# deep-art-project/Music

Measured on AMD Instinct MI355X. Metric: audio samples/sec trained (whole node), 30-layer WaveNet @16kHz, higher is better.
Workload: dtype f32 (forward + recompute: f16 2-term split operands, 2^-22 per element; backward products: bf16 2-term split, 2^-17 per element, f32 range; 3 MFMA per product, f32 accumulate)

## Files before the change

### include/wavenet_hip.h

```cpp
#ifndef WAVENET_HIP_H
#define WAVENET_HIP_H
#include <stdint.h>
#ifdef __cplusplus
extern "C" {
#endif

typedef void* wn_stream_t;
enum { WN_F16X3 = 0, WN_F16X1 = 1, WN_BF16X3 = 2, WN_BF16X1 = 3 };
#define WN_ABI_VERSION 5
#define WN_CE_NUM_PARTIALS 1024

int wn_version(void);
const char* wn_last_error(void);

int wn_pack_weights(const float* flat, const int32_t* idx, uint16_t* out, int n, int mode,
                    wn_stream_t stream);

int wn_chan_gemm(const float* in0, const float* in1, int64_t in_bstride, int in_pitch, int in_lo, int in_hi,
                 int shift0, int shift1, int ks0, int ks1, const uint16_t* wpack, int mt, int m_valid,
                 float* out, int64_t out_bstride, int out_pitch, int out_shift, const float* bias,
                 const float* resid, int64_t resid_bstride, int resid_pitch, int resid_lo,
                 const float* mask, int64_t mask_bstride, int mask_pitch,
                 int t_lo, int t_hi, int relu_in, int batch, int mode, wn_stream_t stream);

int wn_resblock_fwd(const float* x_in, float* x_out, float* z_out, int64_t x_bstride, int64_t z_bstride,
                    int pitch, const uint16_t* wfg, const uint16_t* wd, const float* bias_f,
                    const float* bias_g, const float* bias_d, int n_f, int n_d, int ch, int d,
                    int t_lo, int t_hi, int z_lo, int write_x, const float* cond, int64_t cond_bstride,
                    int cond_pitch, int cond_mode, int cond_le, int cond_q, const uint16_t* cond_pack,
                    int64_t cond_pack_bstride, const uint8_t* cond_idx, int64_t z_half_stride, int batch, int mode,
                    wn_stream_t stream);

int wn_resblock_bwd(const float* x_in, const float* dy, const float* dz, float* dfg, float* z,
                    int64_t x_bstride, int64_t dz_bstride, int64_t dfg_bstride, int64_t z_bstride,
                    int pitch, const uint16_t* wfg, const uint16_t* wdT, const float* bias_f,
                    const float* bias_g, int n_f, int ch, int d, int t_lo, int t_hi, int z_lo,
                    const float* cond, int64_t cond_bstride, int cond_pitch, int cond_mode, int cond_le, int cond_q,
                    int batch, int mode_fwd, int mode_bwd, wn_stream_t stream);

int wn_skip_epilogue_fwd(const float* z, int64_t z_bstride, int pitch, int ks_skip, const uint16_t* w_skip, const float* bias_skip,
                         float* u, float* h, int64_t s_bstride, const uint16_t* w_p1c, const float* bias_p1,
                         const uint16_t* w_p2c, const float* bias_p2, float* o, int64_t o_bstride, int o_pitch,
// ... 26 lines not shown
int wn_resblock_bwd_ms_slabs(int t_lo, int t_hi, int batch);

#define WN_COND_IDX_PAD 64
int wn_resblock_bwd_pq(const float* x_in, const float* p_in, const float* q_in, int dn, int p_lo, const float* dz,
                       float* p_out, float* q_out, int64_t x_bstride, int64_t dz_bstride, int pitch, const uint16_t* wfg,
                       const uint16_t* wdT, const uint16_t* wpq, int ch, int d, int t_lo, int t_hi, int z_lo,
                       float* slab_fg, float* slab_d, const float* cond, int64_t cond_bstride, int cond_pitch, int cond_le,
                       const uint8_t* cond_idx, float* cslab, int64_t dz_half_stride, int chain, int batch, int mode_fwd,
                       int mode_bwd, wn_stream_t stream);
int wn_resblock_bwd_pq_chain_ok(int t_lo, int t_hi, int batch, int d);
int wn_resblock_bwd_pq_slabs(int t_lo, int t_hi, int batch, int d, int chain);
int wn_resblock_bwd_pq_chain_items(int t_lo, int t_hi, int batch, int d, int wg, int* out, int cap);
int wn_resblock_bwd_pq_cond_floats(int t_lo, int t_hi, int batch);
int wn_resblock_bwd_pq_cond_reduce(const float* cslab, const int64_t* slab_off, const int* t_lo, int n_launches, int t_hi, int batch,
                                   int cond_le, float* out, int64_t out_lstride, int64_t out_bstride, int out_pitch,
                                   wn_stream_t stream);
int wn_gate_fwd(const float* fg, int64_t fg_bstride, int dp, int rows, float* z, int64_t z_bstride, int pitch, int t_lo, int t_hi,
                int batch, wn_stream_t stream);
int wn_gate_bwd(const float* fg, int64_t fg_bstride, int dp, int rows, const float* dz, int64_t dz_bstride, float* dfg,
                int64_t dfg_bstride, int pitch, int t_lo, int t_hi, int batch, wn_stream_t stream);
int wn_chunk_softmax_fwd(const float* x, float* y, int64_t nrows, int q, wn_stream_t stream);
int wn_chunk_softmax_bwd(const float* y, const float* dy, float* dx, int64_t nrows, int q, wn_stream_t stream);
int wn_chunk_softmax_ce(const float* x, const int64_t* target, float* probs, float* dx, float* loss_part, int64_t nrows, int q,
                        float inv_n, wn_stream_t stream);
int wn_split16(const float* x, uint16_t* hi, uint16_t* lo, int64_t n, int is_bf16, wn_stream_t stream);
int wn_shift_add(const float* p, const float* q, float* out, int64_t bstride, int pitch, int rows, int dn, int p_lo,
                 int t_lo, int t_hi, int batch, wn_stream_t stream);

int wn_wgrad(const float* a, int64_t a_bstride, int a_pitch, int a_shift, int a_cols,
             const float* b0, const float* b1, int64_t b_bstride, int b_pitch, int b_shift0,
             int b_shift1, int b_cols, int nt_per_tap, int mt, int relu_b, float* c, int ldc,
             int64_t c_slab_stride, int t_lo, int t_hi, int chunk, int batch, int mode, wn_stream_t stream);
int wn_wgrad_slabs(int t_lo, int t_hi, int chunk, int batch);
int wn_causal_wgrad_codes(const int32_t* codes, int scrambled, const float* dx, const float* dx_q, int dn, int p_lo,
                          int64_t dx_bstride, int pitch, int ch, int q, int t, int batch, float* slab, wn_stream_t stream);
int wn_causal_wgrad_codes_slabs(int t, int batch);
int wn_causal_fwd_codes(const int32_t* codes, int scrambled, const float* wt, const float* bias, int n_rows, float* x0,
                        int64_t x_bstride, int pitch, int ch, int q, int t, int batch, wn_stream_t stream);
int wn_reduce_slabs(const int64_t* desc, int n_ops, int64_t total_vec, const float* slab, float* out,
                    wn_stream_t stream);

int wn_bias_grad(const float* a, int64_t a_bstride, int a_pitch, int a_shift, int rows, int t_lo,
                 int t_hi, int batch, float* out, wn_stream_t stream);

int wn_chunk_softmax256_fwd(const float* x, float* y, int64_t nrows, wn_stream_t stream);
int wn_chunk_softmax256_bwd(const float* y, const float* dy, float* dx, int64_t nrows, wn_stream_t stream);
int wn_chunk_softmax256_ce(const float* x, const int64_t* target, float* probs, float* dx,
                           float* loss_part, int64_t nrows, float inv_n, wn_stream_t stream);

int wn_adam_flat(float* p, const float* g, float* m, float* v, int64_t n, float lr, float beta1,
                 float beta2, float eps, float bias_corr1, float bias_corr2, float gscale,
                 wn_stream_t stream);
int wn_sgd_flat(float* p, const float* g, float* momentum_buf, int64_t n, float lr, float momentum, float gscale,
                int first_step, wn_stream_t stream);
int wn_rmsprop_flat(float* p, const float* g, float* square_avg, float* momentum_buf, int64_t n, float lr, float alpha,
                    float eps, float momentum, float gscale, wn_stream_t stream);
int wn_coll_available(void);
int wn_comm_unique_id(char* id128);
int wn_comm_create(int nranks, int rank, const char* id128, void** comm);
int wn_comm_destroy(void* comm);
int wn_allreduce_flat(void* comm, float* buf, int64_t n, wn_stream_t stream);
int wn_gather_grads(const float* packed, const int32_t* idx, float* flat_grad, int n, wn_stream_t stream);
int wn_gather_grads2(const float* packed, const int32_t* idx, const int32_t* idx2, float* flat_grad, int n, wn_stream_t stream);

int wn_cond_expand(const float* tab, int64_t tab_bstride, int tab_pitch, int rows, int t_lo, int t_hi, int mode, int le, int q,
                   float* out, int64_t out_bstride, int out_pitch, int batch, wn_stream_t stream);
// ... 44 lines not shown
```

### music_amd/_lib.py

```python
import ctypes
import os

_HERE = os.path.dirname(os.path.abspath(__file__))
LIB_PATH = os.environ.get("WAVENET_HIP_LIB") or os.path.join(_HERE, "libwavenet_hip.so")

F16X3, F16X1, BF16X3, BF16X1 = 0, 1, 2, 3
MODE_NAMES = {"f16x3": F16X3, "f16x1": F16X1, "bf16x3": BF16X3, "bf16x1": BF16X1}
CE_NUM_PARTIALS = 1024
ABI_VERSION = 5

_p = ctypes.c_void_p
_i = ctypes.c_int
_l = ctypes.c_int64
_f = ctypes.c_float

SIGNATURES = {
    "wn_version": [],
    "wn_pack_weights": [_p, _p, _p, _i, _i, _p],
    "wn_chan_gemm": [_p, _p, _l, _i, _i, _i, _i, _i, _i, _i, _p, _i, _i,
                     _p, _l, _i, _i, _p,
                     _p, _l, _i, _i,
                     _p, _l, _i,
                     _i, _i, _i, _i, _i, _p],
    "wn_skip_epilogue_fwd": [_p, _l, _i, _i, _p, _p, _p, _p, _l, _p, _p, _p, _p, _p, _l, _i, _i, _i, _i, _i, _i, _i, _p],
    "wn_skip_epilogue_bwd": [_p, _l, _i, _p, _p, _l, _i, _p, _p, _p, _l, _p, _p, _p, _i, _i, _i, _i, _i, _i, _i, _p],
    "wn_resblock_fwd": [_p, _p, _p, _l, _l, _i, _p, _p, _p, _p, _p, _i, _i, _i, _i,
                        _i, _i, _i, _i, _p, _l, _i, _i, _i, _i, _p, _l, _p, _l, _i, _i, _p],
    "wn_enc_resblock_fwd": [_p, _p, _p, _l, _l, _i, _p, _p, _p, _p, _i, _i, _i, _i, _i, _i, _i, _i, _p],
    "wn_enc_resblock_bwd": [_p, _p, _p, _p, _l, _l, _l, _i, _p, _i, _i, _i, _i, _i, _p, _p, _i, _i, _p],
    "wn_enc_resblock_bwd_slabs": [_i, _i, _i],
    "wn_enc_resblock_bwd_pq": [_p, _p, _p, _i, _i, _p, _p, _p, _l, _l, _i, _p, _p, _i, _i, _i, _i, _p, _p, _i, _i, _i, _p],
    "wn_avgpool": [_p, _l, _i, _i, _i, _i, _i, _p, _l, _i, _i, _p],
    "wn_resblock_bwd": [_p, _p, _p, _p, _p, _l, _l, _l, _l, _i, _p, _p, _p, _p, _i, _i, _i, _i, _i, _i,
                        _p, _l, _i, _i, _i, _i, _i, _i, _i, _p],
    "wn_cond_expand": [_p, _l, _i, _i, _i, _i, _i, _i, _i, _p, _l, _i, _i, _p],
    "wn_cond_grad": [_p, _l, _i, _i, _i, _i, _i, _i, _i, _p, _l, _i, _i, _p],
    "wn_avgpool_bwd": [_p, _l, _i, _i, _i, _i, _i, _p, _l, _i, _i, _i, _p],
    "wn_wgrad": [_p, _l, _i, _i, _i, _p, _p, _l, _i, _i, _i, _i, _i, _i, _i, _p, _i,
                 _l, _i, _i, _i, _i, _i, _p],
    "wn_wgrad_slabs": [_i, _i, _i, _i],
    "wn_resblock_bwd_ms": [_p, _p, _p, _p, _l, _l, _l, _i, _p, _p, _p, _p, _i, _i, _i, _i, _i, _i, _p, _p,
                           _p, _l, _i, _i, _i, _i, _i, _i, _i, _p],
    "wn_resblock_bwd_ms_slabs": [_i, _i, _i],
    "wn_resblock_bwd_pq": [_p, _p, _p, _i, _i, _p, _p, _p, _l, _l, _i, _p, _p, _p, _i, _i, _i, _i, _i, _p, _p,
                           _p, _l, _i, _i, _p, _p, _l, _i, _i, _i, _i, _p],
    "wn_resblock_bwd_pq_chain_ok": [_i, _i, _i, _i],
    "wn_resblock_bwd_pq_slabs": [_i, _i, _i, _i, _i],
    "wn_resblock_bwd_pq_chain_items": [_i, _i, _i, _i, _i, _p, _i],
    "wn_resblock_bwd_pq_cond_floats": [_i, _i, _i],
    "wn_resblock_bwd_pq_cond_reduce": [_p, _p, _p, _i, _i, _i, _i, _p, _l, _l, _i, _p],
    "wn_split16": [_p, _p, _p, _l, _i, _p],
    "wn_shift_add": [_p, _p, _p, _l, _i, _i, _i, _i, _i, _i, _i, _p],
    "wn_causal_wgrad_codes": [_p, _i, _p, _p, _i, _i, _l, _i, _i, _i, _i, _i, _p, _p],
    "wn_causal_wgrad_codes_slabs": [_i, _i],
    "wn_causal_fwd_codes": [_p, _i, _p, _p, _i, _p, _l, _i, _i, _i, _i, _i, _p],
    "wn_reduce_slabs": [_p, _i, _l, _p, _p, _p],
    "wn_bias_grad": [_p, _l, _i, _i, _i, _i, _i, _i, _p, _p],
    "wn_chunk_softmax256_fwd": [_p, _p, _l, _p],
    "wn_chunk_softmax256_bwd": [_p, _p, _p, _l, _p],
    "wn_chunk_softmax256_ce": [_p, _p, _p, _p, _p, _l, _f, _p],
    "wn_gate_fwd": [_p, _l, _i, _i, _p, _l, _i, _i, _i, _i, _p],
    "wn_gate_bwd": [_p, _l, _i, _i, _p, _l, _p, _l, _i, _i, _i, _i, _p],
    "wn_chunk_softmax_fwd": [_p, _p, _l, _i, _p],
    "wn_chunk_softmax_bwd": [_p, _p, _p, _l, _i, _p],
    "wn_chunk_softmax_ce": [_p, _p, _p, _p, _p, _l, _i, _f, _p],
    "wn_adam_flat": [_p, _p, _p, _p, _l, _f, _f, _f, _f, _f, _f, _f, _p],
    "wn_sgd_flat": [_p, _p, _p, _l, _f, _f, _f, _i, _p],
    "wn_rmsprop_flat": [_p, _p, _p, _p, _l, _f, _f, _f, _f, _f, _p],
    "wn_coll_available": [],
    "wn_comm_unique_id": [_p],
    "wn_comm_create": [_i, _i, _p, _p],
    "wn_comm_destroy": [_p],
    "wn_allreduce_flat": [_p, _p, _l, _p],
# ... 79 lines not shown
              "own setting)" % (torch.get_num_threads(), n, "the container's CPU quota of %d" % q if q is not None else
                                "%d CPUs" % (os.cpu_count() or 1), lw), file=sys.stderr)
        torch.set_num_threads(n)


def load():
    global _lib
    if _lib is not None:
        return _lib
    if not os.path.exists(LIB_PATH):
        raise WavenetHipError(
            "libwavenet_hip.so not found at %s - build it with `python -c 'import __graft_entry__ as g; "
            "g.build()'` or `make -C music_amd/csrc`; there is no CPU fallback" % LIB_PATH)
    import torch
    lib = ctypes.CDLL(LIB_PATH)
    for name, args in SIGNATURES.items():
        fn = getattr(lib, name)
        fn.argtypes = args
        fn.restype = ctypes.c_int
    lib.wn_decode_sync_granules.restype = ctypes.c_int64
    lib.wn_last_error.argtypes = []
    lib.wn_last_error.restype = ctypes.c_char_p
    if lib.wn_version() != ABI_VERSION:
        raise WavenetHipError("libwavenet_hip.so ABI version %d != expected %d" % (lib.wn_version(), ABI_VERSION))
    _lib = lib
    respect_cpu_quota()
    return lib


def wgrad_slabs(t_lo, t_hi, chunk, batch):
    return load().wn_wgrad_slabs(t_lo, t_hi, chunk, batch)


def causal_codes_slabs(t, batch):
    return load().wn_causal_wgrad_codes_slabs(t, batch)


COND_IDX_PAD = 64


def ms_slabs(t_lo, t_hi, batch):
    return load().wn_resblock_bwd_ms_slabs(t_lo, t_hi, batch)


def pq_chain_ok(t_lo, t_hi, batch, d):
    return bool(load().wn_resblock_bwd_pq_chain_ok(t_lo, t_hi, batch, d))


def pq_slabs(t_lo, t_hi, batch, d, chain):
    return load().wn_resblock_bwd_pq_slabs(t_lo, t_hi, batch, d, 1 if chain else 0)


def enc_slabs(t_lo, t_hi, batch):
    return load().wn_enc_resblock_bwd_slabs(t_lo, t_hi, batch)


def decode_sync_granules(n_layers, D, S):
    return int(load().wn_decode_sync_granules(n_layers, D, S))


def call(name, *args):
    lib = load()
    rc = getattr(lib, name)(*args)
    if rc != 0:
        raise WavenetHipError("%s failed (%d): %s" % (name, rc, lib.wn_last_error().decode()))

# ... 25 lines not shown
```

### music_amd/csrc/wn_api.hip

```cpp
#include <stdio.h>
#include <stdlib.h>
#include <string.h>
#include "../../include/wavenet_hip.h"
#include "wn_common.h"
#include "wn_kernels.h"

static_assert(WN_COND_IDX_PAD == WN_PQ_IDX_PAD, "public and kernel-side pad of the bucket bytes differ");
static thread_local char g_err[512] = "";

int wn_set_error(hipError_t e, const char* file, int line) {
    snprintf(g_err, sizeof(g_err), "HIP error %d (%s) at %s:%d", (int)e, hipGetErrorString(e), file, line);
    return -1;
}
int wn_tile_origin(int t_lo) { return t_lo & ~63; }

int wn_num_cus() {
    static std::atomic<int> cus{0};
    int v = cus.load(std::memory_order_relaxed);
    if (v > 0) return v;
    int dev = 0;
    hipDeviceProp_t pr;
    if (hipGetDevice(&dev) != hipSuccess || hipGetDeviceProperties(&pr, dev) != hipSuccess || pr.multiProcessorCount <= 0) return 256;
    cus.store(pr.multiProcessorCount, std::memory_order_relaxed);
    return pr.multiProcessorCount;
// ... 138 lines not shown
                    int batch, int mode_fwd, int mode_bwd, wn_stream_t stream) {
    if (pitch % 4 != 0) return wn_set_error_msg(-4, "wn_resblock_bwd: pitch must be a multiple of 4");
    if (batch > 0 && t_hi > t_lo) {
        WN_REQUIRE("wn_resblock_bwd", x_in, dz, dfg, wfg);
        if (dy) WN_REQUIRE("wn_resblock_bwd", wdT);
    }
    WnResBwdArgs a;
    memset(&a, 0, sizeof(a));
    a.x_in = x_in; a.dy = dy; a.dz = dz; a.dfg = dfg; a.z = z;
    a.x_bstride = x_bstride; a.dz_bstride = dz_bstride; a.dfg_bstride = dfg_bstride; a.z_bstride = z_bstride; a.pitch = pitch;
    a.wfg = wfg; a.wdT = wdT; a.bias_f = bias_f; a.bias_g = bias_g; a.n_f = n_f;
    a.d = d; a.t_lo = t_lo; a.t_hi = t_hi; a.z_lo = z_lo;
    a.cond = cond; a.cond_bstride = cond_bstride; a.cond_pitch = cond_pitch; a.cond_mode = cond_mode;
    a.cond_le = cond_le; a.cond_q = cond_q;
    return wn_launch_resblock_bwd(a, ch, batch, mode_fwd, mode_bwd, (hipStream_t)stream);
}

int wn_wgrad(const float* a_, int64_t a_bstride, int a_pitch, int a_shift, int a_cols,
             const float* b0, const float* b1, int64_t b_bstride, int b_pitch, int b_shift0,
             int b_shift1, int b_cols, int nt_per_tap, int mt, int relu_b, float* c, int ldc,
             int64_t c_slab_stride, int t_lo, int t_hi, int chunk, int batch, int mode, wn_stream_t stream) {
    if (c_slab_stride < (int64_t)mt * 16 * ldc) return wn_set_error_msg(-4, "wn_wgrad: slab stride smaller than C");
    if (batch > 0 && t_hi > t_lo) WN_REQUIRE("wn_wgrad", a_, b0, c);
    WnWgradArgs a;
    memset(&a, 0, sizeof(a));
    a.a = a_; a.a_bstride = a_bstride; a.a_pitch = a_pitch; a.a_shift = a_shift; a.a_cols = a_cols;
    a.b0 = b0; a.b1 = b1; a.b_bstride = b_bstride; a.b_pitch = b_pitch; a.b_shift0 = b_shift0; a.b_shift1 = b_shift1; a.b_cols = b_cols;
    a.nt_per_tap = nt_per_tap; a.mt = mt; a.relu_b = relu_b; a.c = c; a.ldc = ldc; a.c_slab_stride = c_slab_stride;
    a.t_lo = t_lo; a.t_hi = t_hi; a.chunk = chunk;
    return wn_launch_wgrad(a, batch, mode, (hipStream_t)stream);
}

int wn_wgrad_slabs(int t_lo, int t_hi, int chunk, int batch) { return wn_wgrad_num_slabs(t_lo, t_hi, chunk, batch); }

int wn_reduce_slabs(const int64_t* desc, int n_ops, int64_t total_vec, const float* slab, float* out, wn_stream_t stream) {
    if (n_ops > 0 && total_vec > 0) WN_REQUIRE("wn_reduce_slabs", desc, slab, out);
    return wn_launch_reduce_slabs(reinterpret_cast<const long*>(desc), n_ops, total_vec, slab, out, (hipStream_t)stream);
}

int wn_bias_grad(const float* a, int64_t a_bstride, int a_pitch, int a_shift, int rows, int t_lo,
                 int t_hi, int batch, float* out, wn_stream_t stream) {
    if (batch > 0 && t_hi > t_lo && rows > 0) WN_REQUIRE("wn_bias_grad", a, out);
    return wn_launch_bias_grad(a, a_bstride, a_pitch, a_shift, rows, t_lo, t_hi, batch, out, (hipStream_t)stream);
}

int wn_chunk_softmax256_fwd(const float* x, float* y, int64_t nrows, wn_stream_t stream) {
    if (nrows > 0) WN_REQUIRE("wn_chunk_softmax256_fwd", x, y);
    return wn_launch_softmax_fwd(x, y, nrows, (hipStream_t)stream);
}
int wn_chunk_softmax256_bwd(const float* y, const float* dy, float* dx, int64_t nrows, wn_stream_t stream) {
    if (nrows > 0) WN_REQUIRE("wn_chunk_softmax256_bwd", y, dy, dx);
    return wn_launch_softmax_bwd(y, dy, dx, nrows, (hipStream_t)stream);
}
int wn_chunk_softmax256_ce(const float* x, const int64_t* target, float* probs, float* dx,
                           float* loss_part, int64_t nrows, float inv_n, wn_stream_t stream) {
    if (nrows > 0) WN_REQUIRE("wn_chunk_softmax256_ce", x, target);
    return wn_launch_softmax_ce(x, target, probs, dx, loss_part, nrows, inv_n, (hipStream_t)stream);
}
int wn_adam_flat(float* p, const float* g, float* m, float* v, int64_t n, float lr, float beta1,
                 float beta2, float eps, float bias_corr1, float bias_corr2, float gscale, wn_stream_t stream) {
    if (n > 0) WN_REQUIRE("wn_adam_flat", p, g, m, v);
    return wn_launch_adam(p, g, m, v, n, lr, beta1, beta2, eps, bias_corr1, bias_corr2, gscale, (hipStream_t)stream);
}
int wn_sgd_flat(float* p, const float* g, float* momentum_buf, int64_t n, float lr, float momentum, float gscale, int first_step,
                wn_stream_t stream) {
    if (momentum != 0.f && !momentum_buf) return wn_set_error_msg(-4, "wn_sgd_flat: momentum needs its buffer");
// ... 317 lines not shown
```

### music_amd/csrc/wn_kernels.h

```cpp
#pragma once
#include <hip/hip_runtime.h>
#include <stdint.h>

enum { WN_MODE_F16X3 = 0, WN_MODE_F16X1 = 1, WN_MODE_BF16X3 = 2, WN_MODE_BF16X1 = 3 };
static inline int wn_mode_is_bf16(int m) { return m >= 2; }
static inline int wn_mode_ns(int m) { return (m & 1) ? 1 : 3; }
static inline size_t wn_frag_halfs(int mode) { return wn_mode_ns(mode) == 3 ? 1024 : 512; }

struct WnGemmArgs {
    const float* in0; const float* in1;
    long in_bstride; int in_pitch; int in_lo, in_hi;
    int shift0, shift1;
    int ks0, ks1;
    const uint16_t* wpack;
    int mt, m_valid;
    float* out; long out_bstride; int out_pitch; int out_shift;
    const float* bias;
    const float* resid; long resid_bstride; int resid_pitch; int resid_lo;
    const float* mask; long mask_bstride; int mask_pitch;
    int t_lo, t_hi, t_base;
    int relu_in;
    int swz;
};
int wn_launch_gemm(const WnGemmArgs& a, int batch, int mode, hipStream_t st);
// ... 110 lines not shown
int wn_launch_split16(const float* x, uint16_t* hi, uint16_t* lo, long n, int is_bf16, hipStream_t st);
int wn_launch_shift_add(const float* p, const float* q, float* out, long bstride, int pitch, int rows, int dn,
                        int p_lo, int t_lo, int t_hi, int batch, hipStream_t st);
int wn_launch_enc_bwd_rw(const WnResMsArgs& a, int ch, int batch, int mode_bwd, hipStream_t st);
int wn_enc_bwd_slabs(int t_lo, int t_hi, int batch);
struct WnEncPqArgs {
    const float* x_in;
    const float* p_in; const float* q_in; int dn, p_lo;
    const float* h; long h_bstride;
    float* p_out; float* q_out;
    long x_bstride; int pitch;
    const uint16_t* wdT; const uint16_t* wpq;
    float* slab_dil; float* slab_d;
    int d, t_lo, t_hi, t_base;
    int steps_per_clip, items_per_wg, batch, swz;
    int chain, ch_s, ch_qn, ch_rm, ch_g, ch_nchain;
};
int wn_launch_enc_bwd_pq(const WnEncPqArgs& a, int ch, int batch, int mode_bwd, hipStream_t st);

struct WnWgradArgs {
    const float* a; long a_bstride; int a_pitch; int a_shift; int a_cols;
    const float* b0; const float* b1; long b_bstride; int b_pitch; int b_shift0, b_shift1; int b_cols;
    int nt_per_tap;
    int mt;
    int relu_b;
    float* c; int ldc;
    long c_slab_stride;
    int t_lo, t_hi, t_base; int chunk;
    int swz;
};
int wn_launch_wgrad(const WnWgradArgs& a, int batch, int mode, hipStream_t st);
int wn_launch_wgrad2(const WnWgradArgs* a1, const WnWgradArgs* a2, int batch, int mode, hipStream_t st);
int wn_wgrad_num_slabs(int t_lo, int t_hi, int chunk, int batch);
int wn_launch_reduce_slabs(const long* desc, int n_ops, long total_vec, const float* slab, float* out, hipStream_t st);

int wn_launch_causal_wgrad_codes(const int32_t* codes, int scrambled, const float* dx, const float* dxq, int dn, int p_lo,
                                 long dx_bstride, int pitch, int ch, int T, int batch, float* slab, hipStream_t st);
int wn_causal_codes_slabs(int T, int batch);
int wn_launch_causal_fwd_codes(const int32_t* codes, int scrambled, const float* wt, const float* bias, int n_rows, float* x0,
                               long x_bstride, int pitch, int ch, int T, int batch, hipStream_t st);

int wn_launch_softmax_fwd(const float* x, float* y, long nrows, hipStream_t st);
int wn_launch_softmax_bwd(const float* y, const float* dy, float* dx, long nrows, hipStream_t st);
#define WN_CE_PARTIALS 1024
int wn_launch_softmax_ce(const float* x, const int64_t* target, float* probs, float* dx,
                         float* loss_part, long nrows, float inv_n, hipStream_t st);
int wn_launch_adam(float* p, const float* g, float* m, float* v, long n, float lr, float b1, float b2,
                   float eps, float bc1, float bc2, float gscale, hipStream_t st);
int wn_launch_sgd(float* p, const float* g, float* buf, long n, float lr, float momentum, float gscale, int first, hipStream_t st);
int wn_launch_rmsprop(float* p, const float* g, float* sq, float* buf, long n, float lr, float alpha, float eps, float momentum,
                      float gscale, hipStream_t st);
int wn_launch_gather_grads(const float* packed, const int32_t* idx, float* flat_grad, int n, hipStream_t st);
int wn_launch_gather_grads2(const float* packed, const int32_t* idx, const int32_t* idx2, float* flat_grad, int n, hipStream_t st);
int wn_launch_onehot(const int32_t* idx, float* out, int batch, int q, int t, int scrambled, hipStream_t st);
int wn_launch_mulaw_encode(const float* audio, const float* thr, uint8_t* codes, long n, hipStream_t st);
int wn_launch_mulaw_decode(const uint8_t* codes, const float* table, float* audio, long n, hipStream_t st);
int wn_launch_mulaw_encode_q(const float* audio, const float* thr, int n_thr, int32_t* codes, long n, hipStream_t st);
int wn_launch_mulaw_decode_q(const int32_t* codes, const float* table, int q, float* audio, long n, hipStream_t st);
int wn_launch_bias_grad(const float* a, long a_bstride, int a_pitch, int a_shift, int rows, int t_lo,
                        int t_hi, int batch, float* out, hipStream_t st);

int wn_launch_cond_expand(const float* tab, long tab_bstride, int tab_pitch, int rows, int t_lo, int t_hi, int mode, int le, int q,
                          float* out, long out_bstride, int out_pitch, int batch, hipStream_t st);
int wn_launch_cond_grad(const float* in, long in_bstride, int in_pitch, int rows, int t_lo, int t_hi, int mode, int le,
                        int q, float* out, long out_bstride, int out_pitch, int batch, hipStream_t st);
int wn_launch_avgpool_bwd(const float* denc, long denc_bstride, int denc_pitch, int t0, int pool, int n_out, int rows,
// ... 46 lines not shown
```

### music_amd/csrc/wn_wgrad.hip

```cpp
#include <type_traits>
#include "wn_common.h"
#include "wn_kernels.h"

struct WgRaw { f32x4 u0, u1; };

__device__ __forceinline__ WgRaw wg_load(const float* row, int col, int ncols) {
    WgRaw r;
    r.u0 = ld4g(row + col, col, 0, ncols);
    r.u1 = ld4g(row + col + 4, col + 4, 0, ncols);
    return r;
}

template <class T, int NS>
__device__ __forceinline__ void wg_frag(Frag<T>& f, const WgRaw& r, int t, int t_lo, int t_hi, bool masked, bool relu) {
    float v[8] = {r.u0[0], r.u0[1], r.u0[2], r.u0[3], r.u1[0], r.u1[1], r.u1[2], r.u1[3]};
    if (masked) {
#pragma unroll
        for (int j = 0; j < 8; ++j)
            if (t + j < t_lo || t + j >= t_hi) v[j] = 0.f;
    }
    if (relu) {
#pragma unroll
        for (int j = 0; j < 8; ++j) v[j] = fmaxf(v[j], 0.f);
    }
// ... 337 lines not shown
                                              hipFuncAttributeMaxDynamicSharedMemorySize, (int)sh); \
                    done[slot].done(dev); } \
                hipLaunchKernelGGL((wgrad_big_k<TT, NN>), g, b, sh, st, k); } while (0)
            switch (mode) {
                case WN_MODE_BF16X3: WN_BIG(BF16, 3, 0); break;
                case WN_MODE_BF16X1: WN_BIG(BF16, 1, 1); break;
                case WN_MODE_F16X3: WN_BIG(F16, 3, 2); break;
                case WN_MODE_F16X1: WN_BIG(F16, 1, 3); break;
                default: return wn_set_error_msg(-2, "wgrad: bad mode");
            }
#undef WN_BIG
            WN_CHECK_LAUNCH();
            return 0;
        }
        pr.p[1] = pr.p[0]; yg[1] = 0; nch[1] = 0;
    }
    pr.y_split = yg[0];
    dim3 g(nch[0] > nch[1] ? nch[0] : nch[1], yg[0] + yg[1], batch), b(512);
    switch (mode) {
        case WN_MODE_BF16X3: hipLaunchKernelGGL((wgrad_k<BF16, 3>), g, b, 0, st, pr); break;
        case WN_MODE_BF16X1: hipLaunchKernelGGL((wgrad_k<BF16, 1>), g, b, 0, st, pr); break;
        case WN_MODE_F16X3: hipLaunchKernelGGL((wgrad_k<F16, 3>), g, b, 0, st, pr); break;
        case WN_MODE_F16X1: hipLaunchKernelGGL((wgrad_k<F16, 1>), g, b, 0, st, pr); break;
        default: return wn_set_error_msg(-2, "wgrad: bad mode");
    }
    WN_CHECK_LAUNCH();
    return 0;
}

int wn_launch_wgrad(const WnWgradArgs& a, int batch, int mode, hipStream_t st) {
    return wn_launch_wgrad2(&a, nullptr, batch, mode, st);
}

__global__ __launch_bounds__(256) void reduce_slabs_k(const long* __restrict__ desc, int n_ops, long total_vec,
                                                      const float* __restrict__ slab, float* __restrict__ out) {
    long v = (long)blockIdx.x * blockDim.x + threadIdx.x;
    if (v >= total_vec) return;
    int lo = 0, hi = n_ops - 1;
    while (lo < hi) {
        int mid = (lo + hi + 1) >> 1;
        if (desc[mid * 6] <= v) lo = mid; else hi = mid - 1;
    }
    const long* d = desc + lo * 6;
    const long e = (v - d[0]) * 4, n = d[5], stride = d[3];
    const int ns = (int)d[2];
    const float* sp = slab + d[1] + e;
    float* op = out + d[4] + e;
    if (e + 3 < n) {
        f32x4 s8[8];
#pragma unroll
        for (int k = 0; k < 8; ++k) s8[k] = f32x4{0.f, 0.f, 0.f, 0.f};
        int i = 0;
        for (; i + 8 <= ns; i += 8) {
            f32x4 t[8];
#pragma unroll
            for (int k = 0; k < 8; ++k) t[k] = ld4u(sp + (size_t)(i + k) * stride);
#pragma unroll
            for (int k = 0; k < 8; ++k) s8[k] += t[k];
        }
        for (; i < ns; ++i) s8[0] += ld4u(sp + (size_t)i * stride);
        const f32x4 s = ((s8[0] + s8[1]) + (s8[2] + s8[3])) + ((s8[4] + s8[5]) + (s8[6] + s8[7]));
        op[0] = s[0]; op[1] = s[1]; op[2] = s[2]; op[3] = s[3];
    } else {
        for (long k = 0; e + k < n; ++k) {
            float s = 0.f;
            for (int i = 0; i < ns; ++i) s += sp[(size_t)i * stride + k];
// ... 13 lines not shown
```

### music_amd/engine.py

```python
import math
import os

import numpy as np
import torch

from . import _lib
from ._lib import call, ptr

SLACK = 64
PAD_BACK = 2048


def _pad(n, m):
    return (n + m - 1) // m * m


def pack_positions(mt, ks, chained):
    m, s, lane, j = np.indices((mt, ks, 64, 8))
    row = 16 * m + (lane & 15)
    q = lane >> 4
    if chained:
        k = 32 * s + 16 * (j >> 2) + 4 * q + (j & 3)
    else:
        k = 32 * s + 8 * q + j
# ... 347 lines not shown
        self.wt_idx = torch.from_numpy(wt.reshape(-1).astype(np.int32)).to(dev)
        self.wt = torch.zeros(2 * Q * CH, dtype=torch.float32, device=dev)

    def pack_weights(self):
        st = _lib.stream()
        call("wn_pack_weights", ptr(self.flat), ptr(self.pk_f_idx), ptr(self.pk_f), self.pk_f_idx.numel(), self.mode_fwd, st)
        call("wn_pack_weights", ptr(self.flat), ptr(self.pk_b_idx), ptr(self.pk_b), self.pk_b_idx.numel(), self.mode_bwd, st)

    def workspace(self, B, T):
        return self._ws.peek(B, T)

    def _make_workspace(self, B, T):
        dev = self.device
        pitch = _pad(T, 256) + 512
        W = T - self.rf + 1

        def buf(rows):
            t = torch.zeros(SLACK + B * rows * pitch + PAD_BACK, dtype=torch.float32, device=dev)
            return t

        ws = dict(B=B, T=T, W=W, pitch=pitch)
        ws["X"] = torch.zeros(SLACK + (self.N + 1) * B * self.CH * pitch + PAD_BACK, dtype=torch.float32, device=dev)
        ws["Z"] = buf(self.N * self.CH)
        ws["U"] = buf(self.SP)
        ws["H"] = buf(self.SP)
        ws["O"] = torch.zeros(B * self.Q * W + PAD_BACK, dtype=torch.float32, device=dev)
        ws["bwd"] = None
        ws["ms"], ws["pq"] = self._use_ms(), self._use_pq()
        ws["pair"] = self.pair_ok and B % 2 == 0
        ws["pair_fwd"] = ws["pair"] and (B // 2) * ((T + 511) // 512) >= 200
        return ws

    def _bwd_workspace(self, ws):
        if ws["bwd"] is not None:
            return ws["bwd"]
        B, pitch, W, dev = ws["B"], ws["pitch"], ws["W"], self.device

        def buf(rows):
            return torch.zeros(SLACK + B * rows * pitch + PAD_BACK, dtype=torch.float32, device=dev)

        bw = dict(dO=torch.zeros(B * self.Q * W + PAD_BACK, dtype=torch.float32, device=dev),
                  dH=buf(self.SP), dU=buf(self.SP), dZ=buf(self.N * self.CH),
                  dX=[buf(self.CH), buf(self.CH)], dfg=[buf(2 * self.CH), buf(2 * self.CH)],
                  zs=[buf(self.CH), buf(self.CH)])
        T, lo = ws["T"], self.rf - 1
        ms = ws["ms"]
        bw["ms"] = ms
        bw["pq"] = ws["pq"]
        pair = bw["pair"] = ws["pair"]
        if bw["pq"] or pair:
            bw["PQ"] = [(buf(self.CH), buf(self.CH)), (buf(self.CH), buf(self.CH))]
        ck = [int(v) for v in os.environ.get("WN_EPI_WGRAD_CHUNKS", "2048,2048,2048").split(",")]
        if "WN_EPI_WGRAD_CHUNKS" not in os.environ:
            span = T - (lo & ~31)

            def even(c):
                n = -(-span // c)
                return -(-(-(-span // n)) // 32) * 32
            ck = [even(c) for c in ck]
        ops = [("p2", lo, T, ck[0]), ("p1", lo, T, ck[1]), ("skip", lo, T, ck[2])]
        Bp = B // 2 if pair else B
        want = os.environ.get("WN_PQ_CHAIN", "1") == "1"
        bw["chain"] = [want and bool(bw["pq"] or pair) and _lib.pq_chain_ok(self.off[i + 1], T, Bp, self.dil[i]) for i in range(self.N)]
        for i in range(self.N):
            if pair:
                ops.append(("fg2_%d" % i, self.off[i + 1], T, (-3, i)))
                if i < self.N - 1:
                    ops.append(("d2_%d" % i, self.off[i + 1], T, (-3, i)))
                continue
            kind = (-3, i) if bw["pq"] else (-1 if ms else 512)
            ops.append(("fg%d" % i, self.off[i + 1], T, kind))
            if i < self.N - 1:
                ops.append(("d%d" % i, self.off[i + 1], T, kind))
        ops.append(("causal", 1, T, 512))
        ops.append(("causal_codes", 1, T, None))
        plan, desc, so, vs = {}, [], 0, 0
        nslab = {}
        for name, t_lo, t_hi, chunk in ops:
            if isinstance(chunk, tuple):
                nslab[name] = _lib.pq_slabs(t_lo, t_hi, Bp, self.dil[chunk[1]], bw["chain"][chunk[1]])
        for name, t_lo, t_hi, chunk in ops:
            go, r, c = self.gp_off["causal" if name == "causal_codes" else name]
            n = r * c
            if chunk is None:
                ns = _lib.causal_codes_slabs(T, B)
            elif isinstance(chunk, tuple):
                ns = nslab[name]
            elif chunk > 0:
                ns = _lib.wgrad_slabs(t_lo, t_hi, chunk, B)
            else:
                ns = _lib.ms_slabs(t_lo, t_hi, B)
            plan[name] = (so, n, chunk, ns, go)
            if name == "causal_codes":
                desc_codes = desc[:-1] + [[desc[-1][0], so, ns, n, go, n]]
            else:
                desc.append([vs, so, ns, n, go, n])
                vs += (n + 3) // 4
            so += ns * n
        bw["slab"] = torch.empty(so, dtype=torch.float32, device=dev)
        bw["slab_plan"], bw["slab_vec"], bw["slab_nops"] = plan, vs, len(desc)
        bw["slab_desc"] = torch.tensor(desc, dtype=torch.int64, device=dev)
        bw["slab_desc_codes"] = torch.tensor(desc_codes, dtype=torch.int64, device=dev)
        ws["bwd"] = bw
        return bw

    def _use_ms(self):
        ok = self.CH == 64 and self.mode_fwd == _lib.F16X3 and self.mode_bwd == _lib.BF16X3
        if self.ms_bwd is None:
            return ok and os.environ.get("WN_MS_BWD", "1") == "1"
        if self.ms_bwd and not ok:
            raise NotImplementedError("ms_bwd needs 64 padded channels and precision (f16x3, bf16x3)")
        return bool(self.ms_bwd)

    def _use_pq(self):
        return self._use_ms() and not self.use_bias and os.environ.get("WN_PQ_BWD", "1") == "1"

    def _x(self, ws, i):
        return ptr(ws["X"], SLACK + i * ws["B"] * self.CH * ws["pitch"])

    def forward_logits(self, x, ws=None, codes=None):
# ... 111 lines not shown
        br = lambda name: ptr(self.pk_b, self.pk_b_off[name])
        fr = lambda name: ptr(self.pk_f, self.pk_f_off[name])
        lo = self.rf - 1
        xb, zb, sb = CH * pitch, N * CH * pitch, SP * pitch
        plan = bw["slab_plan"]

        def wgrad(name, *args):
            so, n, chunk = plan[name][:3]
            head, (ldc, t_lo, t_hi) = args[:-3], args[-3:]
            call("wn_wgrad", *head, ptr(bw["slab"], so), ldc, n, t_lo, t_hi, chunk, B, mb, st)
        dO, dH, dU, dZ = ptr(bw["dO"]), ptr(bw["dH"], SLACK), ptr(bw["dU"], SLACK), ptr(bw["dZ"], SLACK)
        U, H, Z = ptr(ws["U"], SLACK), ptr(ws["H"], SLACK), ptr(ws["Z"], SLACK)
        main = torch.cuda.current_stream()
        overlap = self.overlap_wgrad
        if overlap and self._side is None:
            self._side = _lib.side_stream(self.device)
        side = self._side if overlap else main

        def on_side(fn):
            if overlap:
                ev = torch.cuda.Event()
                ev.record(main)
                side.wait_event(ev)
            with torch.cuda.stream(side):
                fn(_lib.stream())

        def wgrad_s(name, *args):
            so, n, chunk = plan[name][:3]
            head, (ldc, t_lo, t_hi) = args[:-3], args[-3:]
            on_side(lambda s2: call("wn_wgrad", *head, ptr(bw["slab"], so), ldc, n, t_lo, t_hi, chunk, B, mb, s2))

        wgrad_s("p2", dO, Q * W, W, -lo, W, H, None, sb, pitch, 0, 0, pitch, SP // 16, Q // 16, 1, SP, lo, T)
        self.fmark("b_wgrad_p2")
        if (self.epi_fused_bwd and SP == 256 and Q == 256 and (N * CH // 16) % 3 == 0 and mb in (_lib.F16X3, _lib.BF16X3)
                and not self.use_bias):
            call("wn_skip_epilogue_bwd", dO, Q * W, W, H, U, sb, pitch, dH, dU, dZ, zb, br("p2T"), br("p1Tc"), br("skipTc"),
                 N * CH // 16, N * CH, self.S, lo, T, B, mb, st)
            self.fmark("b_fused")
            wgrad_s("p1", dH, sb, pitch, 0, pitch, U, None, sb, pitch, 0, 0, pitch, SP // 16, SP // 16, 1, SP, lo, T)
            order = os.environ.get("WN_EPI_BWD_ORDER", "1")
            if order == "1":
                wgrad("skip", dU, sb, pitch, 0, pitch, Z, None, zb, pitch, 0, 0, pitch, N * CH // 16, SP // 16, 0, N * CH, lo, T)
            else:
                wgrad_s("skip", dU, sb, pitch, 0, pitch, Z, None, zb, pitch, 0, 0, pitch, N * CH // 16, SP // 16, 0, N * CH, lo, T)
            if order == "1" and overlap:
                ev = torch.cuda.Event()
                ev.record(side)
                main.wait_event(ev)
            self.mark("epilogue_bwd")
            return self._backward_stack(ws, bw, st, main, side, overlap, plan, wgrad)
        call("wn_chan_gemm", dO, None, Q * W, W, 0, W, -lo, 0, Q // 32, 0, br("p2T"), SP // 16, self.S,
             dH, sb, pitch, 0, None, None, 0, 0, 0, H, sb, pitch, lo, T, 0, B, mb, st)
        self.fmark("b_p2T")
        wgrad_s("p1", dH, sb, pitch, 0, pitch, U, None, sb, pitch, 0, 0, pitch, SP // 16, SP // 16, 1, SP, lo, T)
        self.fmark("b_wgrad_p1")
        call("wn_chan_gemm", dH, None, sb, pitch, lo, T, 0, 0, SP // 32, 0, br("p1T"), SP // 16, self.S,
             dU, sb, pitch, 0, None, None, 0, 0, 0, U, sb, pitch, lo, T, 0, B, mb, st)
        self.fmark("b_p1T")
        wgrad_s("skip", dU, sb, pitch, 0, pitch, Z, None, zb, pitch, 0, 0, pitch, N * CH // 16, SP // 16, 0, N * CH, lo, T)
        self.fmark("b_wgrad_skip")
        call("wn_chan_gemm", dU, None, sb, pitch, lo, T, 0, 0, SP // 32, 0, br("skipT"), N * CH // 16, N * CH,
             dZ, zb, pitch, 0, None, None, 0, 0, 0, None, 0, 0, lo, T, 0, B, mb, st)
        if self.use_bias:
            bo = self.gp_bias_off
            call("wn_bias_grad", dO, Q * W, W, -lo, Q, lo, T, B, ptr(self.gpack, bo["post_process_2.bias"]), st)
            call("wn_bias_grad", dH, sb, pitch, 0, self.S, lo, T, B, ptr(self.gpack, bo["post_process_1.bias"]), st)
            for i in range(N):
                call("wn_bias_grad", dU, sb, pitch, 0, self.S, lo, T, B,
                     ptr(self.gpack, bo["dilation_layer_stack.%d.bias" % (4 * i + 3)]), st)
        self.mark("epilogue_bwd")
        return self._backward_stack(ws, bw, st, main, side, overlap, plan, wgrad)

    def _backward_stack(self, ws, bw, st, main, side, overlap, plan, wgrad):
        B, T, W, pitch = ws["B"], ws["T"], ws["W"], ws["pitch"]
        CH, N, SP, Q, mb, mf = self.CH, self.N, self.SP, self.Q, self.mode_bwd, self.mode_fwd
        br = lambda name: ptr(self.pk_b, self.pk_b_off[name])
        fr = lambda name: ptr(self.pk_f, self.pk_f_off[name])
        lo = self.rf - 1
        xb, zb, sb = CH * pitch, N * CH * pitch, SP * pitch
        ev_w = [None, None]
        ev_prev = None
        for i in range(N - 1, -1, -1):
            d = self.dil[i]
            t_lo = self.off[i + 1]
            k = i % 2
            dfg, zs = ptr(bw["dfg"][k], SLACK), ptr(bw["zs"][k], SLACK)
            dy = ptr(bw["dX"][(i + 1) % 2], SLACK) if i < N - 1 else None
            bn = "dilation_layer_stack.%d.bias"
            if overlap and ev_w[k] is not None:
                main.wait_event(ev_w[k])
            if bw["pq"] or bw["pair"]:
                p_out, q_out = (ptr(t, SLACK) for t in bw["PQ"][i % 2])
                chain = 1 if bw["chain"][i] else 0
                if i == 0 and chain:
                    p_out = ptr(bw["dX"][0], SLACK)
                if i < N - 1:
                    p_in, q_in = (ptr(t, SLACK) for t in bw["PQ"][(i + 1) % 2])
                    dn, p_lo = self.dil[i + 1], self.off[i + 2]
                    if bw["chain"][i + 1]:
                        q_in, dn, p_lo = None, 0, t_lo
                else:
                    p_in = q_in = None
                    dn = p_lo = 0
                if bw["pair"]:
# ... 169 lines not shown
```

Baseline: 31.51 million.

## Add dedicated skip-weight-gradient kernel with staged Z tiles and side-stream launch

Adds a specialised wgrad kernel for the skip projection (256 rows of dU times N*CH rows of Z). It stages split Z fragments in double-buffered shared memory and keeps 4x15 MFMA accumulators per wave, with its own chunk-length heuristic sized to the CU count. The fused epilogue backward now uses this kernel and by default issues it on the side stream, where before it ran through the generic wgrad path. The per-thread accumulator count is large, so register pressure and spilling are a risk, and the workspace is rebuilt when the fused-path condition changes.

```diff
diff --git a/include/wavenet_hip.h b/include/wavenet_hip.h
--- a/include/wavenet_hip.h
+++ b/include/wavenet_hip.h
@@ -7,7 +7,7 @@
 
 typedef void* wn_stream_t;
 enum { WN_F16X3 = 0, WN_F16X1 = 1, WN_BF16X3 = 2, WN_BF16X1 = 3 };
-#define WN_ABI_VERSION 5
+#define WN_ABI_VERSION 6
 #define WN_CE_NUM_PARTIALS 1024
 
 int wn_version(void);
@@ -100,6 +100,10 @@
              int b_shift1, int b_cols, int nt_per_tap, int mt, int relu_b, float* c, int ldc,
              int64_t c_slab_stride, int t_lo, int t_hi, int chunk, int batch, int mode, wn_stream_t stream);
 int wn_wgrad_slabs(int t_lo, int t_hi, int chunk, int batch);
+int wn_skip_wgrad(const float* du, int64_t du_bstride, const float* z, int64_t z_bstride, int pitch, int nz, float* c, int ldc,
+                  int64_t c_slab_stride, int t_lo, int t_hi, int chunk, int batch, int mode, wn_stream_t stream);
+int wn_skip_wgrad_chunk(int t_lo, int t_hi, int nz, int batch);
+int wn_skip_wgrad_slabs(int t_lo, int t_hi, int chunk, int batch);
 int wn_causal_wgrad_codes(const int32_t* codes, int scrambled, const float* dx, const float* dx_q, int dn, int p_lo,
                           int64_t dx_bstride, int pitch, int ch, int q, int t, int batch, float* slab, wn_stream_t stream);
 int wn_causal_wgrad_codes_slabs(int t, int batch);
diff --git a/music_amd/_lib.py b/music_amd/_lib.py
--- a/music_amd/_lib.py
+++ b/music_amd/_lib.py
@@ -7,7 +7,7 @@
 F16X3, F16X1, BF16X3, BF16X1 = 0, 1, 2, 3
 MODE_NAMES = {"f16x3": F16X3, "f16x1": F16X1, "bf16x3": BF16X3, "bf16x1": BF16X1}
 CE_NUM_PARTIALS = 1024
-ABI_VERSION = 5
+ABI_VERSION = 6
 
 _p = ctypes.c_void_p
 _i = ctypes.c_int
@@ -39,6 +39,9 @@
     "wn_wgrad": [_p, _l, _i, _i, _i, _p, _p, _l, _i, _i, _i, _i, _i, _i, _i, _p, _i,
                  _l, _i, _i, _i, _i, _i, _p],
     "wn_wgrad_slabs": [_i, _i, _i, _i],
+    "wn_skip_wgrad": [_p, _l, _p, _l, _i, _i, _p, _i, _l, _i, _i, _i, _i, _i, _p],
+    "wn_skip_wgrad_chunk": [_i, _i, _i, _i],
+    "wn_skip_wgrad_slabs": [_i, _i, _i, _i],
     "wn_resblock_bwd_ms": [_p, _p, _p, _p, _l, _l, _l, _i, _p, _p, _p, _p, _i, _i, _i, _i, _i, _i, _p, _p,
                            _p, _l, _i, _i, _i, _i, _i, _i, _i, _p],
     "wn_resblock_bwd_ms_slabs": [_i, _i, _i],
@@ -184,6 +187,14 @@
     return load().wn_wgrad_slabs(t_lo, t_hi, chunk, batch)
 
 
+def skip_wgrad_chunk(t_lo, t_hi, nz, batch):
+    return load().wn_skip_wgrad_chunk(t_lo, t_hi, nz, batch)
+
+
+def skip_wgrad_slabs(t_lo, t_hi, chunk, batch):
+    return load().wn_skip_wgrad_slabs(t_lo, t_hi, chunk, batch)
+
+
 def causal_codes_slabs(t, batch):
     return load().wn_causal_wgrad_codes_slabs(t, batch)
 
diff --git a/music_amd/csrc/wn_api.hip b/music_amd/csrc/wn_api.hip
--- a/music_amd/csrc/wn_api.hip
+++ b/music_amd/csrc/wn_api.hip
@@ -194,6 +194,28 @@
 }
 
 int wn_wgrad_slabs(int t_lo, int t_hi, int chunk, int batch) { return wn_wgrad_num_slabs(t_lo, t_hi, chunk, batch); }
+
+int wn_skip_wgrad(const float* du, int64_t du_bstride, const float* z, int64_t z_bstride, int pitch, int nz, float* c, int ldc,
+                  int64_t c_slab_stride, int t_lo, int t_hi, int chunk, int batch, int mode, wn_stream_t stream) {
+    if (batch <= 0 || t_hi <= t_lo) return 0;
+    WN_REQUIRE("wn_skip_wgrad", du, z, c);
+    if (pitch % 4 != 0) return wn_set_error_msg(-4, "wn_skip_wgrad: pitch must be a multiple of 4");
+    if (nz <= 0 || nz % 16 != 0) return wn_set_error_msg(-4, "wn_skip_wgrad: nz must be a positive multiple of 16");
+    if (t_lo < 0 || t_hi > pitch) return wn_set_error_msg(-4, "wn_skip_wgrad: [t_lo, t_hi) must lie inside the row pitch");
+    if (du_bstride < (int64_t)256 * pitch || z_bstride < (int64_t)nz * pitch)
+        return wn_set_error_msg(-4, "wn_skip_wgrad: clip stride smaller than the clip's rows");
+    if (ldc < nz || c_slab_stride < (int64_t)256 * ldc) return wn_set_error_msg(-4, "wn_skip_wgrad: slab smaller than C");
+    if (chunk < 32 || chunk % 32 != 0) return wn_set_error_msg(-4, "wn_skip_wgrad: chunk must be a positive multiple of 32");
+    WnSkipWgradArgs a;
+    memset(&a, 0, sizeof(a));
+    a.du = du; a.du_bstride = du_bstride; a.z = z; a.z_bstride = z_bstride; a.pitch = pitch; a.nz = nz;
+    a.c = c; a.ldc = ldc; a.c_slab_stride = c_slab_stride; a.t_lo = t_lo; a.t_hi = t_hi; a.chunk = chunk;
+    return wn_launch_skip_wgrad(a, batch, mode, (hipStream_t)stream);
+}
+
+int wn_skip_wgrad_chunk(int t_lo, int t_hi, int nz, int batch) { return wn_skip_wgrad_chunk_len(t_lo, t_hi, nz, batch); }
+
+int wn_skip_wgrad_slabs(int t_lo, int t_hi, int chunk, int batch) { return wn_skip_wgrad_num_slabs(t_lo, t_hi, chunk, batch); }
 
 int wn_reduce_slabs(const int64_t* desc, int n_ops, int64_t total_vec, const float* slab, float* out, wn_stream_t stream) {
     if (n_ops > 0 && total_vec > 0) WN_REQUIRE("wn_reduce_slabs", desc, slab, out);
diff --git a/music_amd/csrc/wn_kernels.h b/music_amd/csrc/wn_kernels.h
--- a/music_amd/csrc/wn_kernels.h
+++ b/music_amd/csrc/wn_kernels.h
@@ -166,6 +166,17 @@
 int wn_launch_wgrad(const WnWgradArgs& a, int batch, int mode, hipStream_t st);
 int wn_launch_wgrad2(const WnWgradArgs* a1, const WnWgradArgs* a2, int batch, int mode, hipStream_t st);
 int wn_wgrad_num_slabs(int t_lo, int t_hi, int chunk, int batch);
+struct WnSkipWgradArgs {
+    const float* du; long du_bstride;
+    const float* z; long z_bstride;
+    int pitch, nz;
+    float* c; int ldc; long c_slab_stride;
+    int t_lo, t_hi, t_base, chunk;
+    int swz;
+};
+int wn_launch_skip_wgrad(const WnSkipWgradArgs& a, int batch, int mode, hipStream_t st);
+int wn_skip_wgrad_chunk_len(int t_lo, int t_hi, int nz, int batch);
+int wn_skip_wgrad_num_slabs(int t_lo, int t_hi, int chunk, int batch);
 int wn_launch_reduce_slabs(const long* desc, int n_ops, long total_vec, const float* slab, float* out, hipStream_t st);
 
 int wn_launch_causal_wgrad_codes(const int32_t* codes, int scrambled, const float* dx, const float* dxq, int dn, int p_lo,
diff --git a/music_amd/csrc/wn_wgrad.hip b/music_amd/csrc/wn_wgrad.hip
--- a/music_amd/csrc/wn_wgrad.hip
+++ b/music_amd/csrc/wn_wgrad.hip
@@ -393,6 +393,166 @@
     return wn_launch_wgrad2(&a, nullptr, batch, mode, st);
 }
 
+#define SKW_NT 15
+#define SKW_MIN_CHUNK 256
+
+template <class T>
+__global__ __launch_bounds__(256) void skip_wgrad_k(WnSkipWgradArgs a) {
+    constexpr int NS = 3, FR = 1024;
+    extern __shared__ __attribute__((aligned(16))) uint16_t l_z[];
+    const int lane = threadIdx.x & 63, wave = threadIdx.x >> 6;
+    const int c = lane & 15, q = lane >> 4;
+    const WnBlock wb = wn_block<true>(a.swz);
+    const int b = wb.z, nb = wb.y;
+    const int tc0 = a.t_base + wb.x * a.chunk;
+    const int tc1 = min(tc0 + a.chunk, a.t_hi);
+    const int ntz = a.nz / 16;
+
+    const float* arow = a.du + (size_t)b * a.du_bstride + (size_t)(64 * wave + c) * a.pitch;
+    const float* zrow[4];
+    bool zval[4];
+#pragma unroll
+    for (int k = 0; k < 4; ++k) {
+        const int slot = wave + 4 * k, nt = nb * SKW_NT + slot;
+        zval[k] = slot < SKW_NT && nt < ntz;
+        zrow[k] = a.z + (size_t)b * a.z_bstride + (size_t)((zval[k] ? nt : 0) * 16 + c) * a.pitch;
+    }
+
+    f32x4 acc[4][SKW_NT];
+#pragma unroll
+    for (int m = 0; m < 4; ++m)
+#pragma unroll
+        for (int n = 0; n < SKW_NT; ++n) acc[m][n] = f32x4{0.f, 0.f, 0.f, 0.f};
+
+    WgRaw ra[4], rz[4];
+    auto ld8 = [&](WgRaw& r, const float* p, int t, bool plain) {
+        if (plain) {
+            r.u0 = ld4u(p);
+            r.u1 = ld4u(p + 4);
+        } else {
+            r.u0 = ld4g(p, t, a.t_lo, tc1);
+            r.u1 = ld4g(p + 4, t + 4, a.t_lo, tc1);
+        }
+    };
+    auto issue_a = [&](int tb) {
+        const int t = tb + 8 * q;
+        const bool plain = tb >= a.t_lo && tb + 32 <= tc1;
+#pragma unroll
+        for (int m = 0; m < 4; ++m) ld8(ra[m], arow + (size_t)(16 * m) * a.pitch + t, t, plain);
+    };
+    auto issue_z = [&](int tb) {
+        const int t = tb + 8 * q;
+        const bool plain = tb >= a.t_lo && tb + 32 <= tc1;
+#pragma unroll
+        for (int k = 0; k < 4; ++k)
+            if (zval[k]) ld8(rz[k], zrow[k] + t, t, plain);
+    };
+    auto frag = [](Frag<T>& f, const WgRaw& r) {
+        const float v[8] = {r.u0[0], r.u0[1], r.u0[2], r.u0[3], r.u1[0], r.u1[1], r.u1[2], r.u1[3]};
+        split8<T, NS>(f, v);
+    };
+    auto park = [&](int stage) {
+#pragma unroll
+        for (int k = 0; k < 4; ++k) {
+            const int slot = wave + 4 * k;
+            if (slot >= SKW_NT) continue;
+            u32x4* dst = reinterpret_cast<u32x4*>(l_z + ((size_t)stage * 16 + slot) * FR);
+            if (!zval[k]) {
+                dst[lane] = u32x4{0u, 0u, 0u, 0u};
+                dst[64 + lane] = u32x4{0u, 0u, 0u, 0u};
+                continue;
+            }
+            Frag<T> f;
+            frag(f, rz[k]);
+            dst[lane] = __builtin_bit_cast(u32x4, f.hi);
+            dst[64 + lane] = __builtin_bit_cast(u32x4, f.lo);
+        }
+    };
+
+    if (tc0 < tc1) {
+        issue_a(tc0);
+        issue_z(tc0);
+        park(0);
+        if (tc0 + 32 < tc1) issue_z(tc0 + 32);
+    }
+    __syncthreads();
+    int it = 0;
+    for (int tb = tc0; tb < tc1; tb += 32, ++it) {
+        const bool more = tb + 32 < tc1;
+        const uint16_t* base = l_z + (size_t)(it & 1) * 16 * FR;
+        Frag<T> af[4], bf[3];
+#pragma unroll
+        for (int m = 0; m < 4; ++m) frag(af[m], ra[m]);
+        if (more) issue_a(tb + 32);
+        load_a<T, NS>(bf[0], base, 0, lane);
+        load_a<T, NS>(bf[1], base, 1, lane);
+#pragma unroll
+        for (int n = 0; n < SKW_NT; ++n) {
+            if (n + 2 < SKW_NT) load_a<T, NS>(bf[(n + 2) % 3], base, n + 2, lane);
+            if (n == 7 && more) {
+                __builtin_amdgcn_sched_barrier(0);
+                park((it + 1) & 1);
+                if (tb + 64 < tc1) issue_z(tb + 64);
+                __builtin_amdgcn_sched_barrier(0);
+            }
+#pragma unroll
+            for (int m = 0; m < 4; ++m) mma<T, NS>(acc[m][n], af[m], bf[n % 3]);
+            __builtin_amdgcn_sched_barrier(0);
+        }
+        __syncthreads();
+    }
+
+    const int n_chunks = (a.t_hi - a.t_base + a.chunk - 1) / a.chunk;
+    float* cs = a.c + ((size_t)b * n_chunks + wb.x) * a.c_slab_stride;
+#pragma unroll
+    for (int n = 0; n < SKW_NT; ++n) {
+        const int nt = nb * SKW_NT + n;
+        if (nt >= ntz) continue;
+#pragma unroll
+        for (int m = 0; m < 4; ++m)
+#pragma unroll
+            for (int i = 0; i < 4; ++i)
+                cs[(size_t)((4 * wave + m) * 16 + 4 * q + i) * a.ldc + nt * 16 + c] = acc[m][n][i];
+    }
+}
+
+int wn_skip_wgrad_chunk_len(int t_lo, int t_hi, int nz, int batch) {
+    if (t_hi <= t_lo || batch <= 0 || nz <= 0) return SKW_MIN_CHUNK;
+    const int span = t_hi - (t_lo & ~31);
+    const int nbk = (nz / 16 + SKW_NT - 1) / SKW_NT;
+    const int nch = max(1, wn_num_cus() / (batch * nbk));
+    int chunk = ((span + nch - 1) / nch + 31) & ~31;
+    return chunk < SKW_MIN_CHUNK ? SKW_MIN_CHUNK : chunk;
+}
+
+int wn_skip_wgrad_num_slabs(int t_lo, int t_hi, int chunk, int batch) {
+    if (t_hi <= t_lo || batch <= 0 || chunk <= 0 || chunk % 32) return 0;
+    return ((t_hi - (t_lo & ~31) + chunk - 1) / chunk) * batch;
+}
+
+int wn_launch_skip_wgrad(const WnSkipWgradArgs& a0, int batch, int mode, hipStream_t st) {
+    if (a0.t_hi <= a0.t_lo || batch <= 0) return 0;
+    if (mode != WN_MODE_F16X3 && mode != WN_MODE_BF16X3) return wn_set_error_msg(-2, "wn_skip_wgrad: x3 modes only");
+    WnSkipWgradArgs a = a0;
+    a.t_base = a.t_lo & ~31;
+    a.swz = wn_xcd_swizzle_enabled();
+    const size_t sh = (size_t)2 * 16 * 1024 * sizeof(uint16_t);
+    int dev = 0;
+    (void)hipGetDevice(&dev);
+    static WnDevOnce done;
+    if (done.need(dev)) {
+        (void)hipFuncSetAttribute(reinterpret_cast<const void*>(&skip_wgrad_k<F16>), hipFuncAttributeMaxDynamicSharedMemorySize, (int)sh);
+        (void)hipFuncSetAttribute(reinterpret_cast<const void*>(&skip_wgrad_k<BF16>), hipFuncAttributeMaxDynamicSharedMemorySize, (int)sh);
+        done.done(dev);
+    }
+    const int nch = (a.t_hi - a.t_base + a.chunk - 1) / a.chunk;
+    const dim3 g(nch, (a.nz / 16 + SKW_NT - 1) / SKW_NT, batch), bl(256);
+    if (mode == WN_MODE_F16X3) hipLaunchKernelGGL(skip_wgrad_k<F16>, g, bl, sh, st, a);
+    else hipLaunchKernelGGL(skip_wgrad_k<BF16>, g, bl, sh, st, a);
+    WN_CHECK_LAUNCH();
+    return 0;
+}
+
 __global__ __launch_bounds__(256) void reduce_slabs_k(const long* __restrict__ desc, int n_ops, long total_vec,
                                                       const float* __restrict__ slab, float* __restrict__ out) {
     long v = (long)blockIdx.x * blockDim.x + threadIdx.x;
diff --git a/music_amd/engine.py b/music_amd/engine.py
--- a/music_amd/engine.py
+++ b/music_amd/engine.py
@@ -403,7 +403,7 @@
         return ws
 
     def _bwd_workspace(self, ws):
-        if ws["bwd"] is not None:
+        if ws["bwd"] is not None and ws["bwd"]["skw"] == self._fused_epi_bwd():
             return ws["bwd"]
         B, pitch, W, dev = ws["B"], ws["pitch"], ws["W"], self.device
 
@@ -429,6 +429,9 @@
                 n = -(-span // c)
                 return -(-(-(-span // n)) // 32) * 32
             ck = [even(c) for c in ck]
+        bw["skw"] = skw = self._fused_epi_bwd()
+        if skw:
+            ck[2] = ((ck[2] + 31) & ~31) if "WN_EPI_WGRAD_CHUNKS" in os.environ else _lib.skip_wgrad_chunk(lo, T, self.N * self.CH, B)
         ops = [("p2", lo, T, ck[0]), ("p1", lo, T, ck[1]), ("skip", lo, T, ck[2])]
         Bp = B // 2 if pair else B
         want = os.environ.get("WN_PQ_CHAIN", "1") == "1"
@@ -457,6 +460,8 @@
                 ns = _lib.causal_codes_slabs(T, B)
             elif isinstance(chunk, tuple):
                 ns = nslab[name]
+            elif name == "skip" and skw:
+                ns = _lib.skip_wgrad_slabs(t_lo, t_hi, chunk, B)
             elif chunk > 0:
                 ns = _lib.wgrad_slabs(t_lo, t_hi, chunk, B)
             else:
@@ -634,17 +639,20 @@
 
         wgrad_s("p2", dO, Q * W, W, -lo, W, H, None, sb, pitch, 0, 0, pitch, SP // 16, Q // 16, 1, SP, lo, T)
         self.fmark("b_wgrad_p2")
-        if (self.epi_fused_bwd and SP == 256 and Q == 256 and (N * CH // 16) % 3 == 0 and mb in (_lib.F16X3, _lib.BF16X3)
-                and not self.use_bias):
+        if self._fused_epi_bwd():
             call("wn_skip_epilogue_bwd", dO, Q * W, W, H, U, sb, pitch, dH, dU, dZ, zb, br("p2T"), br("p1Tc"), br("skipTc"),
                  N * CH // 16, N * CH, self.S, lo, T, B, mb, st)
             self.fmark("b_fused")
             wgrad_s("p1", dH, sb, pitch, 0, pitch, U, None, sb, pitch, 0, 0, pitch, SP // 16, SP // 16, 1, SP, lo, T)
-            order = os.environ.get("WN_EPI_BWD_ORDER", "1")
+            order = os.environ.get("WN_EPI_BWD_ORDER", "0")
+            so, n, chunk = plan["skip"][:3]
+
+            def skip_wgrad(s2):
+                call("wn_skip_wgrad", dU, sb, Z, zb, pitch, N * CH, ptr(bw["slab"], so), N * CH, n, lo, T, chunk, B, mb, s2)
             if order == "1":
-                wgrad("skip", dU, sb, pitch, 0, pitch, Z, None, zb, pitch, 0, 0, pitch, N * CH // 16, SP // 16, 0, N * CH, lo, T)
+                skip_wgrad(st)
             else:
-                wgrad_s("skip", dU, sb, pitch, 0, pitch, Z, None, zb, pitch, 0, 0, pitch, N * CH // 16, SP // 16, 0, N * CH, lo, T)
+                on_side(skip_wgrad)
             if order == "1" and overlap:
                 ev = torch.cuda.Event()
                 ev.record(side)
@@ -672,6 +680,10 @@
                      ptr(self.gpack, bo["dilation_layer_stack.%d.bias" % (4 * i + 3)]), st)
         self.mark("epilogue_bwd")
         return self._backward_stack(ws, bw, st, main, side, overlap, plan, wgrad)
+
+    def _fused_epi_bwd(self):
+        return (self.epi_fused_bwd and self.SP == 256 and self.Q == 256 and (self.N * self.CH // 16) % 3 == 0
+                and self.mode_bwd in (_lib.F16X3, _lib.BF16X3) and not self.use_bias)
 
     def _backward_stack(self, ws, bw, st, main, side, overlap, plan, wgrad):
         B, T, W, pitch = ws["B"], ws["T"], ws["W"], ws["pitch"]
```

Result: no change. 31.38 million (median of 2 runs) (-0.4%).
